# RandomMike1280/AlphaZero-Reversi

Hardware: AMD Instinct MI355X
Metric: self-play board-steps/sec @ 800 sims/move, 8x8 Reversi (higher is better)
Workload: dtype u64 rules + f32 NN (fp32 as 2-part f16 split on MFMA)

## Files before the change

alphazero-reversi_amd/csrc/rvz_engine.hip:

```cpp
#include <hip/hip_bf16.h>
#include <hip/hip_runtime.h>
#include <math.h>
#include <stdint.h>
#include <stdio.h>
#include <stdlib.h>
#include <string.h>

#include <string>
#include <vector>

#include "../../include/rvz.h"
#include "rvz_h2.hip.h"
#include "rvz_pow.hip.h"
#include "rvz_rules.hip.h"
#include "rvz_trace.h"

using namespace rvz;

namespace {

constexpr int WAVE = 64;
constexpr int WPB = 4;
constexpr int PATH_CAP = 64;
constexpr int RNG_DRAWS = 64;
// ... 1501 lines not shown
int rvz_search_visits(rvz_engine* e, int32_t* out) {
    if (!e || !out) return RVZ_EINVAL;
    int r = flush_pending(e);
    if (r != RVZ_OK) return r;
    dim3 grid(grid_games(e->v.G)), block(WPB * WAVE);
    if (e->BS == 8) hipLaunchKernelGGL(k_visits<8>, grid, block, 0, e->stream, e->v, out);
    else hipLaunchKernelGGL(k_visits<6>, grid, block, 0, e->stream, e->v, out);
    return launch_check(e, "k_visits");
}

int rvz_search_compact(rvz_engine* e, int32_t on) {
    if (!e) return RVZ_EINVAL;
    if (e->pending || (e->searching && e->next_batch > 0)) {
        e->err = "rvz_search_compact inside a search";
        return RVZ_EINVAL;
    }
    if (on && !e->live_buf) {
        const size_t nlive = (size_t)e->E * e->v.NS * RVZ_LIVE_PITCH;
        const size_t words = (nlive + e->v.G + 1) / 2 * 2 + 2;
        e->live_buf = dalloc<int32_t>(e, words);
        if (!e->live_buf) { e->err = "hipMalloc failed (live counts)"; return RVZ_ENOMEM; }
        RVZ_HIP(hipMemsetAsync(e->live_buf, 0, sizeof(int32_t) * words, e->stream), e);
        e->live_total = reinterpret_cast<unsigned long long*>(e->live_buf + words - 2);
        e->live_dirty = 0;
    }
    e->v.live = on ? e->live_buf : nullptr;
    e->v.row_of = on ? e->live_buf + (size_t)e->E * e->v.NS * RVZ_LIVE_PITCH : nullptr;
    e->v.live_total = on ? e->live_total : nullptr;
    return RVZ_OK;
}

static int memo_grow(rvz_engine* e) {
    const int M2 = 1 + 2 * e->E * e->NSQ;
    if (e->M == M2) return RVZ_OK;
    const size_t G = e->v.G;
    Node* nodes = nullptr;
    uint32_t* meta = nullptr;
    if (hipMalloc(reinterpret_cast<void**>(&nodes), G * M2 * sizeof(Node)) != hipSuccess ||
        hipMalloc(reinterpret_cast<void**>(&meta), G * M2 * sizeof(uint32_t)) != hipSuccess) {
        if (nodes) (void)hipFree(nodes);
        e->err = "hipMalloc failed (the memo's second node-pool half)";
        return RVZ_ENOMEM;
    }
    RVZ_HIP(hipStreamSynchronize(e->stream), e);
    for (void*& p : e->allocs) {
        if (p == e->v.nodes) { (void)hipFree(p); p = nodes; }
        else if (p == e->v.meta) { (void)hipFree(p); p = meta; }
    }
    e->v.nodes = nodes;
    e->v.meta = meta;
    e->M = e->v.M = M2;
    RVZ_HIP(hipMemsetAsync(meta, 0, G * M2 * sizeof(uint32_t), e->stream), e);
    return RVZ_OK;
}

int rvz_search_memo(rvz_engine* e, int32_t on) {
    if (!e) return RVZ_EINVAL;
    if (e->pending || (e->searching && e->next_batch > 0)) {
        e->err = "rvz_search_memo inside a search";
        return RVZ_EINVAL;
    }
    if (on) {
        const int r = memo_grow(e);
        if (r != RVZ_OK) return r;
    }
    e->v.memo = 1;
    if (memo_drop(e) != RVZ_OK) return RVZ_EHIP;
    e->v.memo = on ? 1 : 0;
    return RVZ_OK;
}

int rvz_search_memo_reset(rvz_engine* e) {
    if (!e) return RVZ_EINVAL;
    const int r = memo_drop(e);
    return r != RVZ_OK ? r : table_bump(e);
}

static bool noise_alpha_ok(double alpha) { return alpha >= 1.0e-37 && alpha <= 3.0e38; }

int rvz_search_root_noise(rvz_engine* e, double alpha, double epsilon, uint32_t salt) {
    if (!e) return RVZ_EINVAL;
    if (!noise_alpha_ok(alpha) || !(epsilon >= 0.0 && epsilon <= 1.0)) {
        e->err = "rvz_search_root_noise: alpha a positive finite float32 (1e-37 .. 3e38), "
                 "0 <= epsilon <= 1";
        return RVZ_EINVAL;
    }
    if (e->pending || (e->searching && e->next_batch > 0)) {
        e->err = "rvz_search_root_noise inside a search";
        return RVZ_EINVAL;
    }
    const float eps = (float)epsilon;
    e->v.noise_eps = eps;
    e->v.noise_om = 1.0f - eps;
    e->v.noise_alpha = (float)alpha;
    e->v.noise_salt = salt;
    return RVZ_OK;
}

int rvz_dirichlet_noise(int32_t bs, int32_t n, const uint64_t* legal, const uint32_t* seed32,
                        const int32_t* tag, uint32_t salt, double alpha, float* out,
                        uint32_t* out_bits, void* stream) {
    if ((bs != 8 && bs != 6) || n < 0 || !noise_alpha_ok(alpha) ||
        (n > 0 && (!legal || !seed32 || !tag || !out)) || ((uintptr_t)out_bits & 15) != 0)
        return RVZ_EINVAL;
    if (n == 0) return RVZ_OK;
    dim3 grid((n + WPB - 1) / WPB), block(WPB * WAVE);
    if (bs == 8) hipLaunchKernelGGL(k_dirichlet<8>, grid, block, 0, (hipStream_t)stream, n, legal, seed32, tag, salt, (float)alpha, out, out_bits);
    else hipLaunchKernelGGL(k_dirichlet<6>, grid, block, 0, (hipStream_t)stream, n, legal, seed32, tag, salt, (float)alpha, out, out_bits);
    return hipGetLastError() == hipSuccess ? RVZ_OK : RVZ_EHIP;
}

int rvz_act_schedule(rvz_engine* e, int32_t from_discs, double late_temperature) {
    if (!e) return RVZ_EINVAL;
    if (from_discs > 0 && !(late_temperature >= 0.0 && late_temperature <= 1.7976931348623157e308)) {
        e->err = "rvz_act_schedule: late_temperature must be finite and >= 0";
        return RVZ_EINVAL;
    }
    if (e->pending || (e->searching && e->next_batch > 0)) {
        e->err = "rvz_act_schedule inside a search";
        return RVZ_EINVAL;
    }
    e->v.sched_from = from_discs > 0 ? from_discs : 0;
    e->v.sched_late = from_discs > 0 ? late_temperature : 0.0;
    return RVZ_OK;
}

int rvz_action_probs(int32_t bs, int32_t n, const int32_t* visits, const double* temperature,
                     const double* u, int32_t* out_idx, double* out_p, int32_t* out_drew,
                     void* stream) {
    if ((bs != 8 && bs != 6) || n < 0 ||
        (n > 0 && (!visits || !temperature || !u || !out_idx || !out_p)))
        return RVZ_EINVAL;
    if (n == 0) return RVZ_OK;
    dim3 grid((n + WPB - 1) / WPB), block(WPB * WAVE);
    if (bs == 8) hipLaunchKernelGGL(k_action_probs<8>, grid, block, 0, (hipStream_t)stream, n, visits, temperature, u, out_idx, out_p, out_drew);
    else hipLaunchKernelGGL(k_action_probs<6>, grid, block, 0, (hipStream_t)stream, n, visits, temperature, u, out_idx, out_p, out_drew);
    return hipGetLastError() == hipSuccess ? RVZ_OK : RVZ_EHIP;
}

int rvz_play_gate(rvz_engine* e, double fraction, double timeout_us, double late_us) {
    if (!e || !(fraction <= 1.0) || !(timeout_us >= 0.0) || !(late_us >= 0.0) ||
        timeout_us > 1e6 || late_us > 1e6) {
        if (e) e->err = "rvz_play_gate: fraction <= 1 (< 0: the default), 0 <= us <= 1e6";
        return RVZ_EINVAL;
    }
    e->gate_frac = fraction;
    e->gate_us = timeout_us;
    e->gate_late_us = late_us;
    return RVZ_OK;
}

int rvz_play_table(rvz_engine* e, int64_t slots, int32_t max_discs) {
    if (!e) return RVZ_EINVAL;
    if (slots != 0 && (slots < 1024 || (slots & (slots - 1)) != 0 || slots > (1ll << 30) ||
                       max_discs < 4)) {
        e->err = "rvz_play_table: slots a power of two in [1024, 2^30] (or 0), max_discs >= 4";
        return RVZ_EINVAL;
    }
    RVZ_HIP(hipStreamSynchronize(e->stream), e);
    if (slots == e->tslots && slots != 0) {
        e->tmaxd = max_discs;
        return table_bump(e);
    }
    table_free(e);
    if (slots == 0) return RVZ_OK;
    const size_t stride = e->BS == 8 ? TabGeo<8>::STRIDE : TabGeo<6>::STRIDE;
    if (hipMalloc(reinterpret_cast<void**>(&e->tab), (size_t)slots * stride * 8) != hipSuccess ||
        hipMalloc(reinterpret_cast<void**>(&e->tclaim), (size_t)slots * 4) != hipSuccess ||
        hipMalloc(reinterpret_cast<void**>(&e->tgen), 4) != hipSuccess) {
        table_free(e);
        e->err = "hipMalloc failed (rvz_play_table)";
        return RVZ_ENOMEM;
    }
    hipError_t st = hipMemset(e->tab, 0, (size_t)slots * stride * 8);
    if (st == hipSuccess) st = hipMemset(e->tclaim, 0, (size_t)slots * 4);
    if (st == hipSuccess) st = hipMemsetD32(e->tgen, 1u, 1);
    if (st == hipSuccess) st = hipDeviceSynchronize();
    if (st != hipSuccess) {
        table_free(e);
        e->err = std::string("rvz_play_table init: ") + hipGetErrorString(st);
        return RVZ_EHIP;
    }
    e->tslots = slots;
    e->tmaxd = max_discs;
    return RVZ_OK;
}

int rvz_search_rows_total(rvz_engine* e, int64_t* out) {
    if (!e || !out) return RVZ_EINVAL;
    *out = 0;
    if (!e->live_total) return RVZ_OK;
    unsigned long long h = 0;
    RVZ_HIP(hipMemcpyAsync(&h, e->live_total, sizeof(h), hipMemcpyDeviceToHost, e->stream), e);
    RVZ_HIP(hipStreamSynchronize(e->stream), e);
    *out = (int64_t)h;
    return RVZ_OK;
}

const int32_t* rvz_search_live_count(const rvz_engine* e) {
    if (!e || !e->v.live || e->next_batch == 0) return nullptr;
    return e->v.live + (size_t)(e->next_batch - 1) * e->v.NS * RVZ_LIVE_PITCH;
}

#ifdef RVZ_WALK_STATS
int rvz_walk_stats(int32_t n_games, int64_t* out10) {
    static std::vector<unsigned int> h;
    const int n = n_games < WALK_STATS_MAX ? n_games : WALK_STATS_MAX;
    h.assign((size_t)n * 5, 0u);
    if (hipMemcpyFromSymbol(h.data(), HIP_SYMBOL(g_walk), h.size() * 4) != hipSuccess)
        return RVZ_EHIP;
    for (int i = 0; i < 10; ++i) out10[i] = 0;
    for (int gi = 0; gi < n; ++gi)
        for (int i = 0; i < 5; ++i) {
            out10[i] += h[(size_t)gi * 5 + i];
            if ((int64_t)h[(size_t)gi * 5 + i] > out10[5 + i]) out10[5 + i] = h[(size_t)gi * 5 + i];
        }
    std::vector<unsigned int> z((size_t)WALK_STATS_MAX * 5, 0u);
    return hipMemcpyToSymbol(HIP_SYMBOL(g_walk), z.data(), z.size() * 4) == hipSuccess
               ? RVZ_OK : RVZ_EHIP;
}

int rvz_walk_times(int32_t n_games, int64_t* out11) {
    static std::vector<unsigned long long> h;
    const int n = n_games < WALK_STATS_MAX ? n_games : WALK_STATS_MAX;
    h.assign((size_t)n * 5, 0ull);
    if (hipMemcpyFromSymbol(h.data(), HIP_SYMBOL(g_wtime), h.size() * 8) != hipSuccess)
        return RVZ_EHIP;
    int best = 0;
    unsigned long long bt = 0;
    double mean[5] = {0, 0, 0, 0, 0};
    for (int gi = 0; gi < n; ++gi) {
        unsigned long long t = 0;
        for (int i = 0; i < 5; ++i) {
            t += h[(size_t)gi * 5 + i];
            mean[i] += (double)h[(size_t)gi * 5 + i] / n;
        }
        if (t > bt) { bt = t; best = gi; }
    }
    for (int i = 0; i < 5; ++i) {
        out11[i] = (int64_t)h[(size_t)best * 5 + i];
        out11[5 + i] = (int64_t)mean[i];
    }
    out11[10] = best;
    std::vector<unsigned long long> z((size_t)WALK_STATS_MAX * 5, 0ull);
    return hipMemcpyToSymbol(HIP_SYMBOL(g_wtime), z.data(), z.size() * 8) == hipSuccess
               ? RVZ_OK : RVZ_EHIP;
}
#endif

#ifdef RVZ_WALK_STATS
int rvz_play_walk_read(int32_t n_games, uint64_t* out) {
    const int n = n_games < WALK_STATS_MAX ? n_games : WALK_STATS_MAX;
    std::vector<unsigned long long> a((size_t)n * 5), b((size_t)n * 4);
    if (hipMemcpyFromSymbol(a.data(), HIP_SYMBOL(g_wtime), a.size() * 8) != hipSuccess ||
        hipMemcpyFromSymbol(b.data(), HIP_SYMBOL(g_ftime), b.size() * 8) != hipSuccess)
        return RVZ_EHIP;
    for (int i = 0; i < n; ++i) {
        for (int k = 0; k < 5; ++k) out[(size_t)i * 9 + k] = a[(size_t)i * 5 + k];
        for (int k = 0; k < 4; ++k) out[(size_t)i * 9 + 5 + k] = b[(size_t)i * 4 + k];
    }
    std::vector<unsigned long long> z((size_t)WALK_STATS_MAX * 5, 0ull);
    if (hipMemcpyToSymbol(HIP_SYMBOL(g_wtime), z.data(), z.size() * 8) != hipSuccess)
        return RVZ_EHIP;
    return hipMemcpyToSymbol(HIP_SYMBOL(g_ftime), z.data(), (size_t)WALK_STATS_MAX * 4 * 8) ==
                   hipSuccess ? RVZ_OK : RVZ_EHIP;
}
#endif

int rvz_search_skip(rvz_engine* e) {
    if (!e) return RVZ_EINVAL;
    const int S = e->cfg.num_simulations, B = e->cfg.batch_size;
    if (!e->searching || e->next_batch == 0 || e->next_batch * B < S) {
        e->err = "rvz_search_skip is only valid after the last rvz_search_step of a search";
        return RVZ_EINVAL;
    }
    if (e->pending) { e->err = "rvz_search_skip after rvz_search_submit"; return RVZ_EINVAL; }
    if (S <= B) {
        e->err = "rvz_search_skip needs a search of at least two batches (num_simulations > "
                 "batch_size): a single batch's leaf is the root";
        return RVZ_EINVAL;
    }
    e->pending = 2;
    return RVZ_OK;
}

int rvz_act(rvz_engine* e, double temperature, const double* u, int32_t apply, int32_t* out_idx,
            double* out_p) {
    const Range trace_range("rvz.act (expand/backup + action + move)");
    if (!e || !out_idx || !out_p) return RVZ_EINVAL;
    const int ex = e->pending;
    dim3 grid(grid_games(e->v.G)), block(WPB * WAVE);
    timing_begin(e, 1);
    if (e->BS == 8) hipLaunchKernelGGL(k_act<8>, grid, block, 0, e->stream, e->v, ex, e->pend_policy, e->pend_is_logits, e->pend_value, temperature, u, apply, out_idx, out_p);
    else hipLaunchKernelGGL(k_act<6>, grid, block, 0, e->stream, e->v, ex, e->pend_policy, e->pend_is_logits, e->pend_value, temperature, u, apply, out_idx, out_p);
    timing_end(e);
    e->pending = 0;
    e->live_dirty = 0;
    if (apply) e->searching = 0;
    return launch_check(e, "k_act");
}

static int64_t play_al4(int64_t n) { return (n + 3) / 4 * 4; }

static int64_t play_qwords(int64_t G) { return 4 + play_al4(G) + 8 * 32; }
int64_t rvz_play_scratch_size(const rvz_engine* e) {
    if (!e) return RVZ_EINVAL;
    const int64_t G = e->v.G;
    return play_qwords(G) + play_al4(G * 3 * e->NSQ) + play_al4(G) + play_al4(G * 192) +
           play_al4(G * e->NPOL) + play_al4(G);
}

#ifndef RVZ_PLAY_GROUP
#define RVZ_PLAY_GROUP 4
#endif
#ifndef RVZ_PLAY_GATE_FRAC
#define RVZ_PLAY_GATE_FRAC 0.8
#endif
#ifndef RVZ_PLAY_GATE_US
#define RVZ_PLAY_GATE_US 400.0
#endif
#ifndef RVZ_PLAY_GATE_LATE_US
#define RVZ_PLAY_GATE_LATE_US 200.0
#endif
extern "C++" {
template <int F, int NB, int CTW, int PTW, int BS, int OCC>
static int play_launch(rvz_engine* e, const View& v, const PlayArgs& pa, int slots_per_cu) {
    int cus = 0;
    if (hipDeviceGetAttribute(&cus, hipDeviceAttributeMultiprocessorCount, e->cfg.device) !=
            hipSuccess || cus <= 0)
        cus = 256;
    PlayArgs a = pa;
    const int slots = cus * slots_per_cu;
    dim3 grid;
    if (a.q_next) {
        if (a.gpw <= 0) a.gpw = RVZ_PLAY_GROUP;
        if (a.gpw > play_gpw_max<F, BS>()) a.gpw = play_gpw_max<F, BS>();
        a.n_groups = (v.G + a.gpw - 1) / a.gpw;
        grid = dim3(a.n_groups < slots ? a.n_groups : slots);
        RVZ_HIP(fill32_async(a.q_next, 0u, (size_t)play_qwords(v.G), e->stream), e);
    } else {
        if (a.gpw <= 0) a.gpw = (v.G + slots - 1) / slots;
        if (a.gpw > play_gpw_max<F, BS>()) a.gpw = play_gpw_max<F, BS>();
        a.n_groups = (v.G + a.gpw - 1) / a.gpw;
        grid = dim3(a.n_groups);
    }
    PlayCtx ctx;
    ctx.v = v;
    ctx.a = a;
    hipLaunchKernelGGL((k_play<F, NB, CTW, PTW, BS, OCC>), grid, dim3(256), 0, e->stream, ctx);
    return launch_check(e, "k_play");
}
}

#ifdef RVZ_PLAY_TIMING
int rvz_play_timing_read(uint64_t* host, int n) {
    if (hipMemcpyFromSymbol(host, HIP_SYMBOL(g_play_t), (size_t)n * 12 * 8) != hipSuccess)
        return RVZ_EHIP;
    if (hipMemcpyFromSymbol(host + (size_t)n * 12, HIP_SYMBOL(g_pass_t), (size_t)n * 6 * 8) !=
        hipSuccess)
        return RVZ_EHIP;
    std::vector<unsigned long long> z((size_t)16384 * 12, 0ull);
    if (hipMemcpyToSymbol(HIP_SYMBOL(g_pass_t), z.data(), (size_t)16384 * 6 * 8) != hipSuccess)
        return RVZ_EHIP;
    return hipMemcpyToSymbol(HIP_SYMBOL(g_play_t), z.data(), z.size() * 8) == hipSuccess
               ? RVZ_OK : RVZ_EHIP;
}
#endif


int rvz_play(rvz_engine* e, const rvz_play_args* a) {
    const Range trace_range("rvz.play (fused search + h2 evaluator)");
    if (!e || !a) return RVZ_EINVAL;
    if (!a->params || !a->blob || !a->scratch || !a->seeds || !a->plies_done || !a->out_idx ||
        !a->out_p || (a->reset && !a->games_done) || a->plies < 1 || a->blocks < 0 ||
        (a->filters != 64 && a->filters != 128 && !(a->filters == 256 && e->BS == 8)) ||
        a->games_per_workgroup < -PLAY_GPW_MAX ||
        e->cfg.leaf_dtype != RVZ_LEAF_F32) {
        e->err = "rvz_play: invalid arguments";
        return RVZ_EINVAL;
    }
    if ((((uintptr_t)a->params | (uintptr_t)a->blob | (uintptr_t)a->scratch) & 15) != 0) {
        e->err = "rvz_play: params, blob and scratch must be 16-byte aligned";
        return RVZ_EINVAL;
    }
    if (e->pending || (e->searching && e->next_batch > 0)) {
        e->err = "rvz_play inside a search";
        return RVZ_EINVAL;
    }
    View v = e->v;
    v.live = nullptr;
    v.row_of = nullptr;
    v.live_total = nullptr;
    v.stats = nullptr;
    const int64_t G = v.G;
    PlayArgs pa;
    pa.prm = a->params;
    pa.L = make_layout(a->filters, a->blocks, e->BS);
    pa.blob = a->blob;
    pa.n_blocks = a->blocks;
    float* sc = a->scratch;
    const bool queue = a->games_per_workgroup <= 0;
    pa.q_next = queue ? reinterpret_cast<unsigned*>(sc) : nullptr;
    pa.q_done = queue ? reinterpret_cast<unsigned*>(sc) + 4 : nullptr;
    pa.n_groups = 0;
    pa.gate = queue ? reinterpret_cast<unsigned long long*>(sc + 4 + play_al4(G)) : nullptr;
    {
        double frac = e->gate_frac, us = e->gate_us, late = e->gate_late_us;
        if (frac < 0.0) {
            frac = RVZ_PLAY_GATE_FRAC;
            us = RVZ_PLAY_GATE_US;
            late = RVZ_PLAY_GATE_LATE_US;
        }
        if (const char* gs = getenv("RVZ_PLAY_GATE")) {
            double f = 0.0, u = 0.0, l = 0.0;
            const int n = sscanf(gs, "%lf,%lf,%lf", &f, &u, &l);
            frac = n >= 2 ? f : 0.0;
            us = u;
            late = n >= 3 ? l : 0.0;
        }
        pa.gate_frac = (queue && frac > 0.0 && us > 0.0)
                           ? (unsigned)(fmin(frac, 1.0) * 65536.0 + 0.5) : 0u;
        pa.gate_t = (unsigned)(us * 100.0);
        pa.gate_late = late > 0.0 ? (unsigned)(late * 100.0) : 0u;
    }
    sc += play_qwords(G);
    pa.x = sc;
    sc += play_al4(G * 3 * e->NSQ);
    pa.need = reinterpret_cast<int32_t*>(sc);
    sc += play_al4(G);
    pa.work = sc;
    sc += play_al4(G * 192);
    pa.logits = sc;
    sc += play_al4(G * e->NPOL);
    pa.value = sc;
    pa.ovf = a->ovf;
    pa.gpw = queue ? -a->games_per_workgroup : a->games_per_workgroup;
    pa.plies = a->plies;
    pa.skip_last = a->skip_last_eval && e->cfg.num_simulations > e->cfg.batch_size ? 1 : 0;
    pa.reset = a->reset ? 1 : 0;
    pa.S = e->cfg.num_simulations;
    pa.B = e->cfg.batch_size;
    pa.temperature = a->temperature;
    pa.seeds = a->seeds;
    pa.stride = a->seed_stride;
    pa.ply_ctr = a->plies_done;
    pa.done = a->games_done;
    pa.out_idx = a->out_idx;
    pa.out_p = a->out_p;
    pa.hist = a->hist;
    pa.rows = reinterpret_cast<unsigned long long*>(a->rows_evaluated);
    pa.budget = a->ply_budget;
    pa.tab = nullptr;
    pa.tclaim = nullptr;
    pa.tgen = nullptr;
    pa.tmask = 0;
    pa.tmaxd = 0;
    pa.tstats = reinterpret_cast<unsigned long long*>(a->table_stats);
    pa.unread = reinterpret_cast<unsigned long long*>(a->rows_unread);
    pa.skip_forced = a->skip_forced_roots && pa.skip_last ? 1 : 0;
    pa.roots_unread = reinterpret_cast<unsigned long long*>(a->roots_unread);
    pa.rec_black = a->rec_black;
    pa.rec_white = a->rec_white;
    pa.rec_side = a->rec_side;
    pa.rec_p = a->rec_p;
    if ((a->rec_black || a->rec_white || a->rec_side || a->rec_p) &&
        !(a->rec_black && a->rec_white && a->rec_side && a->rec_p)) {
        e->err = "rvz_play: rec_black, rec_white, rec_side and rec_p go together";
        return RVZ_EINVAL;
    }
    if (e->tab) {
        if (e->tab_blob != a->blob) {
            if (e->tab_blob) {
                hipStreamCaptureStatus cs = hipStreamCaptureStatusNone;
                if (hipStreamIsCapturing(e->stream, &cs) == hipSuccess &&
                    cs != hipStreamCaptureStatusNone) {
                    e->err = "rvz_play: another weight blob than the table's while the stream is "
                             "capturing (play once eagerly with this evaluator before capturing)";
                    return RVZ_EINVAL;
                }
                const int r = table_bump(e);
                if (r != RVZ_OK) return r;
            }
            e->tab_blob = a->blob;
        }
        pa.tab = e->tab;
        pa.tclaim = e->tclaim;
        pa.tgen = e->tgen;
        pa.tmask = (unsigned)(e->tslots - 1);
        pa.tmaxd = e->tmaxd;
    }
    pa.spin_limit = 1u << 26;
    if (const char* sl = getenv("RVZ_PLAY_SPIN_LIMIT")) pa.spin_limit = (unsigned)strtoul(sl, nullptr, 10);
    e->searching = 0;
    if (e->BS == 8)
        return a->filters == 64    ? play_launch<64, 2, 2, 4, 8, 2>(e, v, pa, 2)
               : a->filters == 128 ? play_launch<128, 1, 2, 4, 8, 2>(e, v, pa, 2)
                                   : play_launch<256, 1, 4, 4, 8, 1>(e, v, pa, 1);
    return a->filters == 64 ? play_launch<64, 3, 2, 4, 6, 2>(e, v, pa, 2)
                            : play_launch<128, 1, 2, 3, 6, 2>(e, v, pa, 2);
}

struct rvz_timer {
    std::vector<hipEvent_t> ev;
};

int rvz_timer_create(int32_t n, rvz_timer** out) {
    if (n <= 0 || !out) return RVZ_EINVAL;
    rvz_timer* t = new rvz_timer;
    t->ev.resize(n, nullptr);
    for (auto& e : t->ev) {
        if (hipEventCreateWithFlags(&e, hipEventDisableSystemFence) != hipSuccess) {
            for (auto& f : t->ev)
                if (f) (void)hipEventDestroy(f);
            delete t;
            return RVZ_EHIP;
        }
    }
    *out = t;
    return RVZ_OK;
}

int rvz_timer_record(rvz_timer* t, int32_t i, void* stream) {
    if (!t || i < 0 || i >= (int32_t)t->ev.size()) return RVZ_EINVAL;
    return hipEventRecord(t->ev[i], (hipStream_t)stream) == hipSuccess ? RVZ_OK : RVZ_EHIP;
}

int rvz_timer_elapsed(rvz_timer* t, int32_t i, int32_t j, float* ms) {
    if (!t || !ms || i < 0 || j < 0 || i >= (int32_t)t->ev.size() || j >= (int32_t)t->ev.size())
        return RVZ_EINVAL;
    if (hipEventSynchronize(t->ev[j]) != hipSuccess) return RVZ_EHIP;
    return hipEventElapsedTime(ms, t->ev[i], t->ev[j]) == hipSuccess ? RVZ_OK : RVZ_EHIP;
}

void rvz_timer_destroy(rvz_timer* t) {
    if (!t) return;
    for (auto& e : t->ev)
        if (e) (void)hipEventDestroy(e);
    delete t;
}

int rvz_counters(const rvz_engine* e, int64_t* out2) {
    if (!e || !out2) return RVZ_EINVAL;
    out2[0] = e->counters[0];
    out2[1] = e->counters[1];
    return RVZ_OK;
}

int rvz_stats_enable(rvz_engine* e, int32_t on) {
    if (!e) return RVZ_EINVAL;
    e->v.stats = on ? e->stats_buf : nullptr;
    if (on) RVZ_HIP(hipMemsetAsync(e->stats_buf, 0, 3 * (size_t)e->v.G * sizeof(unsigned long long), e->stream), e);
    return RVZ_OK;
}

int rvz_stats_read(rvz_engine* e, int64_t* out3) {
    if (!e || !out3) return RVZ_EINVAL;
    const size_t G = e->v.G;
    std::vector<unsigned long long> h(3 * G);
    RVZ_HIP(hipMemcpyAsync(h.data(), e->stats_buf, h.size() * sizeof(unsigned long long),
                           hipMemcpyDeviceToHost, e->stream), e);
    RVZ_HIP(hipStreamSynchronize(e->stream), e);
    for (int k = 0; k < 3; ++k) {
        unsigned long long t = 0;
        for (size_t g = 0; g < G; ++g) t += h[k * G + g];
        out3[k] = (int64_t)t;
    }
    return RVZ_OK;
}

int rvz_timing_enable(rvz_engine* e, int32_t on) {
    if (!e) return RVZ_EINVAL;
    e->timing = on ? 1 : 0;
    e->ev_used = 0;
    e->ev_marks.clear();
    return RVZ_OK;
}

int rvz_timing_read(rvz_engine* e, double* out_ms, int32_t* out_n) {
    if (!e || !out_ms || !out_n) return RVZ_EINVAL;
    RVZ_HIP(hipStreamSynchronize(e->stream), e);
    double sum[2] = {0.0, 0.0};
    int32_t n[2] = {0, 0};
    for (const auto& mk : e->ev_marks) {
        float ms = 0.0f;
        RVZ_HIP(hipEventElapsedTime(&ms, e->ev_pool[mk.second], e->ev_pool[mk.second + 1]), e);
        sum[mk.first] += ms;
        n[mk.first] += 1;
    }
    for (int k = 0; k < 2; ++k) {
        out_ms[k] = n[k] ? sum[k] / n[k] : 0.0;
        out_n[k] = n[k];
    }
    return RVZ_OK;
}

int rvz_tree_nodes(const rvz_engine* e) { return e ? e->M : RVZ_EINVAL; }

int rvz_tree_export(rvz_engine* e, void* nodes_out, uint32_t* meta_out) {
    if (!e) return RVZ_EINVAL;
    int r = flush_pending(e);
    if (r != RVZ_OK) return r;
    const size_t n = (size_t)e->v.G * e->M;
    if (nodes_out) RVZ_HIP(hipMemcpyAsync(nodes_out, e->v.nodes, n * sizeof(Node), hipMemcpyDeviceToDevice, e->stream), e);
    if (meta_out) RVZ_HIP(hipMemcpyAsync(meta_out, e->v.meta, n * sizeof(uint32_t), hipMemcpyDeviceToDevice, e->stream), e);
    return RVZ_OK;
}

int rvz_footprint(const rvz_engine* e, int64_t* bytes_tree, int64_t* bytes_env) {
    if (!e) return RVZ_EINVAL;
    const int64_t G = e->v.G;
    if (bytes_tree)
        *bytes_tree = G * e->M * (int64_t)(sizeof(Node) + sizeof(uint32_t)) +
                      G * (PATH_CAP * 4 + 4 * 4 + 8) + G * (4 + 2 * e->E * 4);
    if (bytes_env) *bytes_env = G * (8 + 8 + 16) + G * (RNG_DRAWS * 8 + 4);
    return RVZ_OK;
}

}
```

alphazero-reversi_amd/csrc/rvz_play.hip.h:

```cpp

struct PlayArgs {
    const float* prm;
    Layout L;
    const uint16_t* blob;
    int n_blocks;
    float* x;
    int32_t* need;
    float* work;
    float* logits;
    float* value;
    float* ovf;
    int gpw, plies, skip_last, reset, S, B;
    double temperature;
    int64_t* seeds;
    int64_t stride;
    int64_t* ply_ctr;
    int64_t* done;
    int32_t* out_idx;
    double* out_p;
    int32_t* hist;
    unsigned long long* rows;
    const int32_t* budget;
    unsigned spin_limit;
    unsigned long long* tab;
    unsigned* tclaim;
    const unsigned* tgen;
    unsigned tmask;
    int tmaxd;
    unsigned long long* tstats;
    unsigned long long* unread;
    uint64_t* rec_black;
    uint64_t* rec_white;
    int32_t* rec_side;
    double* rec_p;
    unsigned* q_next;
    unsigned* q_done;
    int n_groups;
    unsigned long long* gate;
    unsigned gate_frac;
    unsigned gate_t;
    unsigned gate_late;
    int skip_forced;
    unsigned long long* roots_unread;
};
constexpr int PLAY_GPW_MAX = 64;
template <int F, int BS>
__host__ __device__ constexpr bool play_heads_lds() { return F == 64 && BS == 8; }
template <int F, int BS>
__host__ __device__ constexpr int play_gpw_max() {
    return play_heads_lds<F, BS>() ? 8 : PLAY_GPW_MAX;
}
enum : int { PF_QUEUED = 1, PF_READY = 2, PF_DONE = 4, PF_EVAL = 8, PF_HELD = 16 };
constexpr int32_t ERR_SCHED = 16;

template <int BS>
struct TabGeo {
    static constexpr int NSQ = Geo<BS>::NSQ;
    static constexpr int NG = NSQ + 8;
    static constexpr int STRIDE = (NG + 7) / 8 * 8;
};
constexpr int TAB_PROBES = 8;

__device__ __forceinline__ uint64_t tab_mix(uint64_t z) {
    z ^= z >> 30;
    z *= 0xbf58476d1ce4e5b9ull;
    z ^= z >> 27;
    z *= 0x94d049bb133111ebull;
    return z ^ (z >> 31);
}
__device__ __forceinline__ uint64_t tab_hash(uint64_t P, uint64_t O, uint64_t V) {
    return tab_mix(P ^ tab_mix(O ^ tab_mix(V + 0x9e3779b97f4a7c15ull)));
}
template <int NSQ>
__device__ __forceinline__ uint32_t tab_key_word(int idx, uint64_t P, uint64_t O, uint64_t V) {
    const int k = idx - (NSQ + 2);
    const uint64_t w = k < 2 ? P : (k < 4 ? O : V);
    return (k & 1) ? (uint32_t)(w >> 32) : (uint32_t)w;
}

template <int BS>
__device__ __forceinline__ int tab_read(const unsigned long long* __restrict__ tab, uint32_t sl,
                                         uint32_t gen, uint64_t P, uint64_t O, uint64_t V,
                                         int lane, uint64_t& x0, uint64_t& x1) {
    using T = TabGeo<BS>;
    constexpr int NSQ = T::NSQ, NG = T::NG;
    const unsigned long long* e = tab + (size_t)sl * T::STRIDE;
    x0 = 0;
    x1 = 0;
    if (lane < NG) x0 = __hip_atomic_load(e + lane, __ATOMIC_RELAXED, __HIP_MEMORY_SCOPE_AGENT);
    if (NG > 64 && lane < NG - 64)
        x1 = __hip_atomic_load(e + 64 + lane, __ATOMIC_RELAXED, __HIP_MEMORY_SCOPE_AGENT);
    bool stale = false, other = false;
    if (lane < NG) {
        stale |= (uint32_t)(x0 >> 32) != gen;
        if (lane >= NSQ + 2) other |= (uint32_t)x0 != tab_key_word<NSQ>(lane, P, O, V);
    }
    if (NG > 64 && lane < NG - 64) {
        stale |= (uint32_t)(x1 >> 32) != gen;
        if (64 + lane >= NSQ + 2) other |= (uint32_t)x1 != tab_key_word<NSQ>(64 + lane, P, O, V);
    }
    if (__ballot(stale) != 0ull) return 0;
    return __ballot(other) != 0ull ? 1 : 2;
}

template <int BS, int IDX>
__device__ __forceinline__ uint32_t tab_datum(uint64_t x0, uint64_t x1) {
    if constexpr (IDX < 64) return (uint32_t)__builtin_amdgcn_readlane((int)(uint32_t)x0, IDX);
    else return (uint32_t)__builtin_amdgcn_readlane((int)(uint32_t)x1, IDX - 64);
}

template <int BS>
__device__ __forceinline__ bool tab_lookup(const PlayArgs& a, uint32_t gen, uint64_t P,
                                           uint64_t O, uint64_t V, int lane, int g) {
    constexpr int NSQ = Geo<BS>::NSQ, NPOL = Geo<BS>::NPOL;
    const uint64_t h = tab_hash(P, O, V);
    for (int i = 0; i < TAB_PROBES; ++i) {
        const uint32_t sl = (uint32_t)(h + i) & a.tmask;
        uint64_t x0, x1;
        const int r = tab_read<BS>(a.tab, sl, gen, P, O, V, lane, x0, x1);
        if (r == 0) return false;
        if (r == 1) continue;
        float* row = a.logits + (size_t)g * NPOL;
        if (lane < NSQ) row[lane] = __uint_as_float((uint32_t)x0);
        if (lane == 0) {
            row[NSQ] = __uint_as_float(tab_datum<BS, NSQ>(x0, x1));
            a.value[g] = __uint_as_float(tab_datum<BS, NSQ + 1>(x0, x1));
        }
        return true;
    }
    return false;
}

template <int BS>
__device__ __forceinline__ int tab_insert(const PlayArgs& a, uint32_t gen, uint64_t P, uint64_t O,
                                          uint64_t V, int lane, int g) {
    using T = TabGeo<BS>;
    constexpr int NSQ = T::NSQ, NPOL = Geo<BS>::NPOL, NG = T::NG;
    const uint64_t h = tab_hash(P, O, V);
    for (int i = 0; i < TAB_PROBES; ++i) {
        const uint32_t sl = (uint32_t)(h + i) & a.tmask;
        uint32_t c = 0;
        if (lane == 0) c = __hip_atomic_load(a.tclaim + sl, __ATOMIC_RELAXED, __HIP_MEMORY_SCOPE_AGENT);
        c = (uint32_t)__builtin_amdgcn_readfirstlane((int)c);
        if (c == gen) {
            uint64_t x0, x1;
            if (tab_read<BS>(a.tab, sl, gen, P, O, V, lane, x0, x1) == 2) return 0;
            continue;
        }
        uint32_t won = 0;
        if (lane == 0) {
            uint32_t expect = c;
            won = __hip_atomic_compare_exchange_strong(a.tclaim + sl, &expect, gen,
                                                       __ATOMIC_RELAXED, __ATOMIC_RELAXED,
                                                       __HIP_MEMORY_SCOPE_AGENT) ? 1u : 0u;
        }
        if (!__builtin_amdgcn_readfirstlane((int)won)) continue;
        const float* row = a.logits + (size_t)g * NPOL;
        const float val = a.value[g];
        unsigned long long* e = a.tab + (size_t)sl * T::STRIDE;
        const unsigned long long tag = (unsigned long long)gen << 32;
        if (lane < NG) {
            const uint32_t d = lane < NPOL ? __float_as_uint(row[lane])
                               : lane == NSQ + 1 ? __float_as_uint(val)
                                                 : tab_key_word<NSQ>(lane, P, O, V);
            __hip_atomic_store(e + lane, tag | d, __ATOMIC_RELAXED, __HIP_MEMORY_SCOPE_AGENT);
        }
        if (NG > 64 && lane < NG - 64) {
            const int idx = 64 + lane;
            const uint32_t d = idx < NPOL ? __float_as_uint(row[idx])
                               : idx == NSQ + 1 ? __float_as_uint(val)
                                                : tab_key_word<NSQ>(idx, P, O, V);
            __hip_atomic_store(e + idx, tag | d, __ATOMIC_RELAXED, __HIP_MEMORY_SCOPE_AGENT);
        }
        return 1;
    }
    return 0;
}

__device__ __forceinline__ void gate_open(unsigned long long* w, unsigned r) {
    unsigned long long v = __hip_atomic_load(w, __ATOMIC_RELAXED, __HIP_MEMORY_SCOPE_AGENT);
    while ((unsigned)(v >> 32) == r) {
        if (__hip_atomic_compare_exchange_strong(w, &v, (unsigned long long)(r + 1u) << 32,
                                                 __ATOMIC_RELAXED, __ATOMIC_RELAXED,
                                                 __HIP_MEMORY_SCOPE_AGENT)) {
            __hip_atomic_store(w + 1, __builtin_amdgcn_s_memrealtime(), __ATOMIC_RELAXED,
                               __HIP_MEMORY_SCOPE_AGENT);
            return;
        }
    }
}
__device__ __forceinline__ unsigned long long* gate_line(unsigned long long* gate) {
    const unsigned x = (unsigned)__builtin_amdgcn_s_getreg((31 << 11) | 20) & 7u;
    return gate + 16 * x;
}
__device__ __forceinline__ void gate_running(unsigned long long* gate, long long d) {
    __hip_atomic_fetch_add(gate_line(gate) + 2, (unsigned long long)d, __ATOMIC_RELAXED,
                           __HIP_MEMORY_SCOPE_AGENT);
}
__device__ __forceinline__ void play_gate(unsigned long long* gate, unsigned frac, unsigned t,
                                          unsigned late) {
    unsigned long long* w = gate_line(gate);
    if (late) {
        const unsigned long long t_open =
            __hip_atomic_load(w + 1, __ATOMIC_RELAXED, __HIP_MEMORY_SCOPE_AGENT);
        if (t_open && __builtin_amdgcn_s_memrealtime() - t_open < late) return;
    }
    const unsigned long long running =
        __hip_atomic_load(w + 2, __ATOMIC_RELAXED, __HIP_MEMORY_SCOPE_AGENT);
    if (running < 4) return;
    const unsigned k = max(1u, (unsigned)((running * frac) >> 16));
    const unsigned long long old =
        __hip_atomic_fetch_add(w, 1ull, __ATOMIC_RELAXED, __HIP_MEMORY_SCOPE_AGENT);
    const unsigned r = (unsigned)(old >> 32);
    if ((unsigned)old + 1u >= k) {
        gate_open(w, r);
        return;
    }
    const unsigned long long t0 = __builtin_amdgcn_s_memrealtime();
    for (;;) {
        __builtin_amdgcn_s_sleep(2);
        const unsigned long long v = __hip_atomic_load(w, __ATOMIC_RELAXED, __HIP_MEMORY_SCOPE_AGENT);
        if ((unsigned)(v >> 32) != r) return;
        if (__builtin_amdgcn_s_memrealtime() - t0 > t) {
            gate_open(w, r);
            return;
        }
    }
}

struct PlayCtx {
    View v;
    PlayArgs a;
};
__device__ __forceinline__ int opaque_tid() {
    int t = threadIdx.x;
    asm volatile("" : "+v"(t));
    return t;
}
__device__ __forceinline__ const PlayCtx& play_ctx() {
    const __attribute__((address_space(4))) char* p =
        (const __attribute__((address_space(4))) char*)__builtin_amdgcn_kernarg_segment_ptr();
    asm volatile("" : "+s"(p));
    return *(const PlayCtx*)p;
}

#ifdef RVZ_PLAY_TIMING
__device__ unsigned long long g_play_t[16384][12];
#define PT_NOW(t) const unsigned long long t = __builtin_amdgcn_s_memtime()
#define PT_ADD(i, v) if (tid == 0 && blockIdx.x < 16384) g_play_t[blockIdx.x][i] += (v)
#else
#define PT_NOW(t)
#define PT_ADD(i, v)
#endif

template <int F, int NBOARD, int CTW, int PTW, int BS, int OCC>
__global__ __launch_bounds__(256) __attribute__((amdgpu_waves_per_eu(OCC, OCC)))
void k_play(PlayCtx ctx0) {
    (void)ctx0;
    using WT = WaveTilesH<F, CTW, PTW>;
    constexpr bool ILV = RVZ_H2_ILV && NBOARD == 2 && BS == 8 && PTW == 4 && WT::CG == 2;
    using GH = GeoH<NBOARD, BS, 64 * CTW * H2_TM / F, ILV>;
    using C = CfgH<F, GH::NPIX>;
    constexpr int NPOL = Geo<BS>::NPOL;
    constexpr bool HLDS = play_heads_lds<F, BS>();
    constexpr int GMAX = play_gpw_max<F, BS>();
    constexpr int HROW = heads_in_floats(BS) / 16;
    constexpr int SP_BYTES = WPB * (NPOL + 7) * 8;
    static_assert(heads_in_floats(BS) * 4 <= C::RMAX, "heads rows fit");
    static_assert(SP_BYTES + WPB * 624 * 4 <= C::RMAX, "act / reset scratch fits");
    __shared__ __attribute__((aligned(16))) char smem[C::BYTES];
    __shared__ int st_k[GMAX];
    __shared__ int st_f[GMAX];
    __shared__ int st_p[GMAX];
    __shared__ uint64_t st_bits[GMAX * 3];
    __shared__ uint64_t q_bits[(GMAX + NBOARD) * 3];
    __shared__ __attribute__((aligned(16))) float hin[HLDS ? GMAX * HROW : 4];
    __shared__ int q_rows[GMAX + 16];
    __shared__ int s_nq;
    __shared__ float vpart[4][16];
    __shared__ int s_task[2];
    __shared__ unsigned s_tgen;
    const int tid = threadIdx.x;
    const int wave = __builtin_amdgcn_readfirstlane(tid >> 6);
    int E, G, gpw, total, queue, task_plies;
    {
        const PlayCtx& c = play_ctx();
        E = c.v.E;
        G = c.v.G;
        gpw = c.a.gpw;
        queue = c.a.q_next != nullptr;
        total = queue ? c.a.n_groups * c.a.plies : 0;
        task_plies = queue ? 1 : c.a.plies;
    }
    bool ovf = false;
    __shared__ unsigned s_cnt[5];
    if (tid < 5) s_cnt[tid] = 0u;
    if (tid == 0) {
        const PlayArgs& a = play_ctx().a;
        s_tgen = a.tab ? __hip_atomic_load(a.tgen, __ATOMIC_RELAXED, __HIP_MEMORY_SCOPE_AGENT) : 0u;
    }
    double* sp = reinterpret_cast<double*>(smem) + wave * (NPOL + 7);
    uint32_t* key = reinterpret_cast<uint32_t*>(smem + SP_BYTES) + wave * 624;
    if constexpr (F >= 128 && BS == 8) {
        const PlayArgs& a = play_ctx().a;
        if (tid == 0 && a.gate_frac > 0) gate_running(a.gate, 1);
    }
    PT_NOW(t_start);
    for (int task_i = 0;; ++task_i) {
        int gi, ply0;
        if (!queue) {
            if (task_i > 0) break;
            gi = blockIdx.x;
            ply0 = 0;
        } else {
            PT_NOW(t_q0);
            if (tid == 0) {
                const PlayCtx& c = play_ctx();
                const PlayArgs& a = c.a;
                const bool failed = __hip_atomic_load(c.v.err, __ATOMIC_RELAXED,
                                                      __HIP_MEMORY_SCOPE_AGENT) & ERR_SCHED;
                const unsigned t =
                    failed ? (unsigned)total
                           : __hip_atomic_fetch_add(a.q_next, 1u, __ATOMIC_RELAXED,
                                                    __HIP_MEMORY_SCOPE_AGENT);
                int tg = -1, tp = 0;
                if ((int)t < total) {
                    tg = (int)(t % (unsigned)a.n_groups);
                    tp = (int)(t / (unsigned)a.n_groups);
                    unsigned spins = 0;
                    while ((int)__hip_atomic_load(a.q_done + tg, __ATOMIC_RELAXED,
                                                  __HIP_MEMORY_SCOPE_AGENT) < tp) {
                        __builtin_amdgcn_s_sleep(4);
                        ++spins;
                        if (spins > a.spin_limit ||
                            ((spins & 1023u) == 0 &&
                             (__hip_atomic_load(c.v.err, __ATOMIC_RELAXED,
                                                __HIP_MEMORY_SCOPE_AGENT) & ERR_SCHED))) {
                            atomicOr(c.v.err, ERR_SCHED);
                            tg = -1;
                            break;
                        }
                    }
                    __builtin_amdgcn_fence(__ATOMIC_ACQUIRE, "agent");
                    asm volatile("s_waitcnt vmcnt(0)" ::: "memory");
                }
                s_task[0] = tg;
                s_task[1] = tp;
            }
            __syncthreads();
            gi = __builtin_amdgcn_readfirstlane(s_task[0]);
            ply0 = __builtin_amdgcn_readfirstlane(s_task[1]);
            if (gi < 0) break;
            PT_NOW(t_q1);
            PT_ADD(8, t_q1 - t_q0);
            PT_ADD(9, 1);
        }
        const int g0 = gi * gpw;
        const int ng = min(gpw, G - g0);
        {
            const int32_t* bud = play_ctx().a.budget;
            for (int j = tid; j < ng; j += 256) {
                st_k[j] = 0;
                st_f[j] = (bud && ply0 >= bud[g0 + j]) ? PF_DONE : 0;
                st_p[j] = 0;
            }
        }
        __syncthreads();
        for (;;) {
            PT_NOW(t_c0);
            for (int j = wave; j < ng; j += WPB) {
                const PlayCtx& c = play_ctx();
                const View& v = c.v;
                const PlayArgs& a = c.a;
                const int lane = opaque_tid() & 63;
                const int g = g0 + j;
                int f = __builtin_amdgcn_readfirstlane(st_f[j]);
                if (f & (PF_QUEUED | PF_DONE)) continue;
                int k = __builtin_amdgcn_readfirstlane(st_k[j]);
                int np = __builtin_amdgcn_readfirstlane(st_p[j]);
                WT_NOW(ft_step);
                FT_CNT();
                for (;;) {
                    unsigned long long ab = 0;
                    if (k < E) {
                        const int first = k == 0;
                        const GameS root = load_game(v, g);
                        uint32_t root_meta = 0, carry = LINK_NONE;
                        int root_n = 0;
                        if (!first) {
                            root_meta = v.meta[(size_t)g * v.M];
                            root_n = v.nodes[(size_t)g * v.M].n;
                        } else if (v.memo) {
                            carry = v.carry[g];
                        }
                        if (f & PF_READY) {
                            WT_NOW(ft_e);
                            const ExpIn x = expand_load<BS>(v, g, lane, a.logits, a.value);
                            const int rn =
                                expand_backup_phase<BS>(v, g, lane, x, 1, &root_meta, ab);
                            if (rn >= 0) root_n = rn;
                            f &= ~PF_READY;
                            FT_ADD(0, ft_e);
                        }
                        const int bsz = min(a.B, a.S - k * a.B);
                        const bool unread = a.skip_last && !first && m_nchild(root_meta) >= E - 1;
                        const Forced fz{first && a.skip_forced ? E : 0, a.S, a.B};
                        const int copies = select_phase<BS, float>(v, g, lane, first, bsz, k, root,
                                                                   root_meta, root_n, carry, a.x,
                                                                   a.need, ab, st_bits + 3 * j,
                                                                   unread, fz);
                        if (copies <= -2) {
                            k = E;
                            const int left = -2 - copies;
                            if (lane == 0) {
                                if (left & 255) atomicAdd(&s_cnt[3], (unsigned)(left & 255));
                                if (left >> 8) atomicAdd(&s_cnt[4], 1u);
                            }
                            continue;
                        }
                        ++k;
                        if (copies < 0 && k < E && lane == 0) atomicAdd(&s_cnt[3], 1u);
                        if (copies > 0 && !(k == E && a.skip_last)) {
                            if (a.tab) {
                                const uint64_t P = st_bits[3 * j], O = st_bits[3 * j + 1],
                                               Vb = st_bits[3 * j + 2];
                                WT_NOW(ft_t);
                                const bool hit = __popcll(P | O) <= a.tmaxd &&
                                                 tab_lookup<BS>(a, s_tgen, P, O, Vb, lane, g);
                                WT_ADD(0, ft_t);
                                if (hit) {
                                    __builtin_amdgcn_fence(__ATOMIC_SEQ_CST, "workgroup");
                                    f |= PF_READY;
                                    if (lane == 0) atomicAdd(&s_cnt[1], 1u);
                                    continue;
                                }
                            }
                            f |= PF_QUEUED;
                            break;
                        }
                        continue;
                    }
                    WT_NOW(ft_a);
                    bool over = false;
                    double* outp = a.out_p;
                    if (a.rec_black) {
                        const size_t ri = (size_t)(ply0 + np) * v.G + g;
                        if (lane == 0) {
                            a.rec_black[ri] = v.black[g];
                            a.rec_white[ri] = v.white[g];
                            a.rec_side[ri] = v.status[(size_t)g * 4];
                        }
                        outp = a.rec_p + (size_t)(ply0 + np) * v.G * Geo<BS>::NPOL;
                    }
                    const int idx = act_game<BS>(v, g, lane, sp, (f & PF_READY) ? 1 : 2,
                                                 a.logits, 1, a.value, a.temperature, nullptr, 1,
                                                 a.out_idx, outp, &over);
                    f &= ~PF_READY;
                    int64_t sd = 0;
                    if (lane == 0) {
                        if (idx >= 0) a.ply_ctr[g] += 1;
                        if (a.hist) a.hist[(size_t)(ply0 + np) * v.G + g] = idx;
                        if (a.reset && over) {
                            a.done[g] += 1;
                            sd = a.seeds[g] + a.stride;
                            a.seeds[g] = sd;
                        }
                    }
                    if (a.reset && over) {
                        sd = __shfl(sd, 0);
                        reset_game<BS>(v, g, lane, (uint32_t)(sd & 0xFFFFFFFFll), key);
                    }
                    FT_ADD(1, ft_a);
                    ++np;
                    k = 0;
                    if (np >= task_plies || (a.budget && ply0 + np >= a.budget[g])) {
                        f |= PF_DONE;
                        break;
                    }
                }
                FT_ADD(2, ft_step);
                if (lane == 0) {
                    st_k[j] = k;
                    st_f[j] = f;
                    st_p[j] = np;
                }
            }
            __syncthreads();
            PT_NOW(t_c1);
            PT_ADD(0, t_c1 - t_c0);
            PT_ADD(4, 1);
            if (tid == 0) {
                int n = 0;
                for (int j = 0; j < ng; ++j)
                    if (st_f[j] & PF_QUEUED) ++n;
                int hold = n > NBOARD ? n % NBOARD : 0;
                for (int j = ng - 1; j >= 0; --j) {
                    const int fj = st_f[j];
                    if (!(fj & PF_QUEUED)) continue;
                    if (hold > 0 && !(fj & PF_HELD)) {
                        st_f[j] = fj | PF_HELD;
                        --hold;
                    } else {
                        st_f[j] = (fj & ~PF_HELD) | PF_EVAL;
                    }
                }
                n = 0;
                for (int j = 0; j < ng; ++j)
                    if (st_f[j] & PF_EVAL) {
                        for (int ch = 0; ch < 3; ++ch) q_bits[3 * n + ch] = st_bits[3 * j + ch];
                        q_rows[n++] = g0 + j;
                    }
                for (int i = n; i < n + 16; ++i) q_rows[i] = -1;
                for (int i = 3 * n; i < 3 * (n + NBOARD); ++i) q_bits[i] = 0;
                s_nq = n;
            }
            __syncthreads();
            const int nq = __builtin_amdgcn_readfirstlane(s_nq);
            if (nq == 0) break;
            if (tid == 0) s_cnt[0] += (unsigned)nq;
            PT_NOW(t_c2);

            for (int p0 = 0; p0 < nq; p0 += NBOARD) {
                if constexpr (F >= 128 && BS == 8) {
                    if (play_ctx().a.gate_frac > 0) {
                        if (tid == 0) {
                            const PlayArgs& a = play_ctx().a;
                            play_gate(a.gate, a.gate_frac, a.gate_t, a.gate_late);
                        }
                        __syncthreads();
                    }
                }
                const PlayArgs& a = play_ctx().a;
                int gb[NBOARD];
#pragma unroll
                for (int k = 0; k < NBOARD; ++k) gb[k] = q_rows[p0 + k];
                const int t = opaque_tid();
                if constexpr (HLDS)
                    h2_pass<F, NBOARD, CTW, PTW, BS>(
                        smem, a.x, gb, q_bits + 3 * p0, a.prm, a.L, a.blob, a.n_blocks,
                        HeadsInLds<BS>{hin, p0, nq}, t, t & 63,
                        __builtin_amdgcn_readfirstlane(t >> 6), ovf);
                else
                    h2_pass<F, NBOARD, CTW, PTW, BS>(
                        smem, a.x, gb, q_bits + 3 * p0, a.prm, a.L, a.blob, a.n_blocks,
                        HeadsGlobalIdx<NBOARD>(a.work, gb), t, t & 63,
                        __builtin_amdgcn_readfirstlane(t >> 6), ovf);
                __syncthreads();
            }
            PT_NOW(t_c3);
            PT_ADD(1, t_c3 - t_c2);
            PT_ADD(5, (nq + NBOARD - 1) / NBOARD);
            PT_ADD(6, nq);
            for (int h0 = 0; h0 < nq; h0 += 16) {
                const PlayArgs& a = play_ctx().a;
                if constexpr (HLDS)
                    heads_fc16<BS, HeadRowsList, false, false, GMAX>(
                        a.work, HeadRowsList{q_rows + h0}, a.prm, a.L, a.logits, a.value, hin,
                        vpart, opaque_tid());
                else
                    heads_fc16<BS, HeadRowsList, false, true>(
                        a.work, HeadRowsList{q_rows + h0}, a.prm, a.L, a.logits, a.value,
                        reinterpret_cast<float*>(smem), vpart, opaque_tid());
            }
            if (play_ctx().a.tab) {
                __syncthreads();
                for (int i = wave; i < nq; i += WPB) {
                    const PlayArgs& a = play_ctx().a;
                    const uint64_t P = q_bits[3 * i], O = q_bits[3 * i + 1], Vb = q_bits[3 * i + 2];
                    if (__popcll(P | O) <= a.tmaxd)
                        if (tab_insert<BS>(a, s_tgen, P, O, Vb, opaque_tid() & 63, q_rows[i]) &&
                            (opaque_tid() & 63) == 0)
                            atomicAdd(&s_cnt[2], 1u);
                }
            }
            for (int j = tid; j < ng; j += 256)
                if (st_f[j] & PF_EVAL) st_f[j] = (st_f[j] & ~(PF_QUEUED | PF_EVAL)) | PF_READY;
            __syncthreads();
            PT_NOW(t_c4);
            PT_ADD(2, t_c4 - t_c3);
        }
        if (queue) {
            asm volatile("s_waitcnt vmcnt(0)" ::: "memory");
            __syncthreads();
            if (tid == 0) {
                __builtin_amdgcn_fence(__ATOMIC_RELEASE, "agent");
                asm volatile("s_waitcnt vmcnt(0)" ::: "memory");
                __hip_atomic_store(play_ctx().a.q_done + gi, (unsigned)(ply0 + 1), __ATOMIC_RELAXED,
                                   __HIP_MEMORY_SCOPE_AGENT);
            }
        }
    }
    if constexpr (F >= 128 && BS == 8) {
        const PlayArgs& a = play_ctx().a;
        if (tid == 0 && a.gate_frac > 0) gate_running(a.gate, -1);
    }
#ifdef RVZ_PLAY_TIMING
    {
        PT_NOW(t_end);
        PT_ADD(3, t_end - t_start);
        if (tid == 0 && blockIdx.x < 16384)
            g_play_t[blockIdx.x][10] = __builtin_amdgcn_s_memrealtime();
        if (tid == 0 && blockIdx.x < 16384)
            g_play_t[blockIdx.x][7] =
                ((unsigned long long)__builtin_amdgcn_s_getreg((31 << 11) | 20) << 32) |
                __builtin_amdgcn_s_getreg((31 << 11) | 4);
    }
#endif
    float* ovw = play_ctx().a.ovf;
    if (ovf && ovw) *ovw = 1.0f;
    unsigned long long* rows = play_ctx().a.rows;
    __syncthreads();
    if (rows && tid == 0) atomicAdd(rows, (unsigned long long)s_cnt[0]);
    unsigned long long* ts = play_ctx().a.tstats;
    if (ts && tid == 0) {
        if (s_cnt[1]) atomicAdd(ts, (unsigned long long)s_cnt[1]);
        if (s_cnt[2]) atomicAdd(ts + 1, (unsigned long long)s_cnt[2]);
    }
    unsigned long long* un = play_ctx().a.unread;
    if (un && tid == 0 && s_cnt[3]) atomicAdd(un, (unsigned long long)s_cnt[3]);
    unsigned long long* ur = play_ctx().a.roots_unread;
    if (ur && tid == 0 && s_cnt[4]) atomicAdd(ur, (unsigned long long)s_cnt[4]);
}
```

Before: 1.729 million.

## Replace ply-ordered ticket queue with claim-based scheduling of ready game groups

Each group's q_done word now packs a published-ply count and a claimed-ply count. Instead of taking the next ticket in ply-major order and spinning until that group finishes its previous ply, a whole wave scans all groups, picks the least-advanced ready group (rotated by block index), and claims it with a CAS. This is meant to remove idle spinning when the ticketed group is still busy while other groups are ready. In exchange it adds per-claim scan cost over all groups, CAS contention between blocks, and a final spin-wait until every group has finished all plies.

```diff
diff --git a/alphazero-reversi_amd/csrc/rvz_engine.hip b/alphazero-reversi_amd/csrc/rvz_engine.hip
--- a/alphazero-reversi_amd/csrc/rvz_engine.hip
+++ b/alphazero-reversi_amd/csrc/rvz_engine.hip
@@ -1827,7 +1827,8 @@
 
 static int64_t play_al4(int64_t n) { return (n + 3) / 4 * 4; }
 
-static int64_t play_qwords(int64_t G) { return 4 + play_al4(G) + 8 * 32; }
+static int64_t play_gwords(int64_t G) { return 2 * play_al4(G); }
+static int64_t play_qwords(int64_t G) { return 4 + play_gwords(G) + 8 * 32; }
 int64_t rvz_play_scratch_size(const rvz_engine* e) {
     if (!e) return RVZ_EINVAL;
     const int64_t G = e->v.G;
@@ -1926,9 +1927,9 @@
     float* sc = a->scratch;
     const bool queue = a->games_per_workgroup <= 0;
     pa.q_next = queue ? reinterpret_cast<unsigned*>(sc) : nullptr;
-    pa.q_done = queue ? reinterpret_cast<unsigned*>(sc) + 4 : nullptr;
+    pa.q_done = queue ? reinterpret_cast<unsigned long long*>(sc + 4) : nullptr;
     pa.n_groups = 0;
-    pa.gate = queue ? reinterpret_cast<unsigned long long*>(sc + 4 + play_al4(G)) : nullptr;
+    pa.gate = queue ? reinterpret_cast<unsigned long long*>(sc + 4 + play_gwords(G)) : nullptr;
     {
         double frac = e->gate_frac, us = e->gate_us, late = e->gate_late_us;
         if (frac < 0.0) {
diff --git a/alphazero-reversi_amd/csrc/rvz_play.hip.h b/alphazero-reversi_amd/csrc/rvz_play.hip.h
--- a/alphazero-reversi_amd/csrc/rvz_play.hip.h
+++ b/alphazero-reversi_amd/csrc/rvz_play.hip.h
@@ -34,7 +34,7 @@
     int32_t* rec_side;
     double* rec_p;
     unsigned* q_next;
-    unsigned* q_done;
+    unsigned long long* q_done;
     int n_groups;
     unsigned long long* gate;
     unsigned gate_frac;
@@ -282,14 +282,13 @@
     __shared__ unsigned s_tgen;
     const int tid = threadIdx.x;
     const int wave = __builtin_amdgcn_readfirstlane(tid >> 6);
-    int E, G, gpw, total, queue, task_plies;
+    int E, G, gpw, queue, task_plies;
     {
         const PlayCtx& c = play_ctx();
         E = c.v.E;
         G = c.v.G;
         gpw = c.a.gpw;
         queue = c.a.q_next != nullptr;
-        total = queue ? c.a.n_groups * c.a.plies : 0;
         task_plies = queue ? 1 : c.a.plies;
     }
     bool ovf = false;
@@ -314,45 +313,81 @@
             ply0 = 0;
         } else {
             PT_NOW(t_q0);
-            if (tid == 0) {
+            if (wave == 0) {
                 const PlayCtx& c = play_ctx();
                 const PlayArgs& a = c.a;
-                const bool failed = __hip_atomic_load(c.v.err, __ATOMIC_RELAXED,
-                                                      __HIP_MEMORY_SCOPE_AGENT) & ERR_SCHED;
-                const unsigned t =
-                    failed ? (unsigned)total
-                           : __hip_atomic_fetch_add(a.q_next, 1u, __ATOMIC_RELAXED,
-                                                    __HIP_MEMORY_SCOPE_AGENT);
+                const int n = a.n_groups;
+                const unsigned plies = (unsigned)a.plies;
+                const int rot = (int)((unsigned long long)blockIdx.x * (unsigned)n / gridDim.x);
                 int tg = -1, tp = 0;
-                if ((int)t < total) {
-                    tg = (int)(t % (unsigned)a.n_groups);
-                    tp = (int)(t / (unsigned)a.n_groups);
-                    unsigned spins = 0;
-                    while ((int)__hip_atomic_load(a.q_done + tg, __ATOMIC_RELAXED,
-                                                  __HIP_MEMORY_SCOPE_AGENT) < tp) {
-                        __builtin_amdgcn_s_sleep(4);
-                        ++spins;
-                        if (spins > a.spin_limit ||
-                            ((spins & 1023u) == 0 &&
-                             (__hip_atomic_load(c.v.err, __ATOMIC_RELAXED,
-                                                __HIP_MEMORY_SCOPE_AGENT) & ERR_SCHED))) {
-                            atomicOr(c.v.err, ERR_SCHED);
-                            tg = -1;
+                bool stop = __hip_atomic_load(c.v.err, __ATOMIC_RELAXED,
+                                              __HIP_MEMORY_SCOPE_AGENT) & ERR_SCHED;
+                unsigned spins = 0;
+                while (!stop) {
+                    unsigned long long best = ~0ull;
+                    bool left = false;
+                    for (int i = tid; i < n; i += 64) {
+                        const unsigned long long w = __hip_atomic_load(
+                            a.q_done + i, __ATOMIC_RELAXED, __HIP_MEMORY_SCOPE_AGENT);
+                        const unsigned pub = (unsigned)(w >> 32), cl = (unsigned)w;
+                        if (cl < plies) {
+                            left = true;
+                            if (cl == pub) {
+                                const int r = i - rot + (i < rot ? n : 0);
+                                const unsigned long long key =
+                                    ((unsigned long long)pub << 32) | (unsigned)r;
+                                best = key < best ? key : best;
+                            }
+                        }
+                    }
+#pragma unroll
+                    for (int off = 32; off > 0; off >>= 1) {
+                        const unsigned long long o = __shfl_xor(best, off, 64);
+                        best = o < best ? o : best;
+                    }
+                    if (best != ~0ull) {
+                        const unsigned p = (unsigned)(best >> 32);
+                        int g = (int)(unsigned)best + rot;
+                        g -= g >= n ? n : 0;
+                        int won = 0;
+                        if (tid == 0) {
+                            unsigned long long want = ((unsigned long long)p << 32) | p;
+                            won = __hip_atomic_compare_exchange_strong(
+                                a.q_done + g, &want, want + 1ull, __ATOMIC_RELAXED,
+                                __ATOMIC_RELAXED, __HIP_MEMORY_SCOPE_AGENT);
+                        }
+                        if (__builtin_amdgcn_readfirstlane(won)) {
+                            tg = g;
+                            tp = (int)p;
                             break;
                         }
-                    }
-                    __builtin_amdgcn_fence(__ATOMIC_ACQUIRE, "agent");
-                    asm volatile("s_waitcnt vmcnt(0)" ::: "memory");
+                        continue;
+                    }
+                    if (__ballot(left) == 0) break;
+                    __builtin_amdgcn_s_sleep(4);
+                    ++spins;
+                    PT_ADD(11, 1);
+                    if (spins > a.spin_limit ||
+                        ((spins & 1023u) == 0 &&
+                         (__hip_atomic_load(c.v.err, __ATOMIC_RELAXED,
+                                            __HIP_MEMORY_SCOPE_AGENT) & ERR_SCHED))) {
+                        if (tid == 0) atomicOr(c.v.err, ERR_SCHED);
+                        stop = true;
+                    }
                 }
-                s_task[0] = tg;
-                s_task[1] = tp;
+                __builtin_amdgcn_fence(__ATOMIC_ACQUIRE, "agent");
+                asm volatile("s_waitcnt vmcnt(0)" ::: "memory");
+                if (tid == 0) {
+                    s_task[0] = tg;
+                    s_task[1] = tp;
+                }
             }
             __syncthreads();
             gi = __builtin_amdgcn_readfirstlane(s_task[0]);
             ply0 = __builtin_amdgcn_readfirstlane(s_task[1]);
-            if (gi < 0) break;
             PT_NOW(t_q1);
             PT_ADD(8, t_q1 - t_q0);
+            if (gi < 0) break;
             PT_ADD(9, 1);
         }
         const int g0 = gi * gpw;
@@ -585,8 +620,11 @@
             if (tid == 0) {
                 __builtin_amdgcn_fence(__ATOMIC_RELEASE, "agent");
                 asm volatile("s_waitcnt vmcnt(0)" ::: "memory");
-                __hip_atomic_store(play_ctx().a.q_done + gi, (unsigned)(ply0 + 1), __ATOMIC_RELAXED,
-                                   __HIP_MEMORY_SCOPE_AGENT);
+                __hip_atomic_fetch_add(play_ctx().a.q_done + gi, 1ull << 32, __ATOMIC_RELAXED,
+                                       __HIP_MEMORY_SCOPE_AGENT);
+                if (ply0 + 1 == play_ctx().a.plies)
+                    __hip_atomic_fetch_add(play_ctx().a.q_next, 1u, __ATOMIC_RELAXED,
+                                           __HIP_MEMORY_SCOPE_AGENT);
             }
         }
     }
@@ -606,6 +644,25 @@
                 __builtin_amdgcn_s_getreg((31 << 11) | 4);
     }
 #endif
+    if (queue && tid == 0) {
+        const PlayCtx& c = play_ctx();
+        const PlayArgs& a = c.a;
+        unsigned spins = 0;
+        bool stop = __hip_atomic_load(c.v.err, __ATOMIC_RELAXED, __HIP_MEMORY_SCOPE_AGENT) &
+                    ERR_SCHED;
+        while (!stop && (int)__hip_atomic_load(a.q_next, __ATOMIC_RELAXED,
+                                               __HIP_MEMORY_SCOPE_AGENT) < a.n_groups) {
+            __builtin_amdgcn_s_sleep(4);
+            ++spins;
+            if (spins > a.spin_limit ||
+                ((spins & 1023u) == 0 &&
+                 (__hip_atomic_load(c.v.err, __ATOMIC_RELAXED, __HIP_MEMORY_SCOPE_AGENT) &
+                  ERR_SCHED))) {
+                atomicOr(c.v.err, ERR_SCHED);
+                stop = true;
+            }
+        }
+    }
     float* ovw = play_ctx().a.ovf;
     if (ovf && ovw) *ovw = 1.0f;
     unsigned long long* rows = play_ctx().a.rows;
```

Measured after the change: 1.793 million, median of 6. +3.7%, better.
